# jianzongwu/betrayed-by-captions

Measured on AMD Instinct MI355X. Metric: images/sec (COCO-shaped 1024x1024, 100 queries, forward-only), higher is better.
Workload: dtype f32; 1 GPU; configs[1]: R50 + 100 queries, 1024x1024, batch 2/GPU, forward-only; global_batch=2, parallelism=replicas x1, precision=fp32 (parity mode, f16x3 MFMA), hip_graph=True, x3_overflow=False, library_fallbacks=0

## Files before the change

betrayed-by-captions_amd/_lib.py:

```python
import ctypes
import os

import torch

_HERE = os.path.dirname(os.path.abspath(__file__))
LIB_PATH = os.path.join(_HERE, 'lib', 'libcgg_hip.so')

CGG_F32 = 0
CGG_BF16 = 1

_c_int = ctypes.c_int
_c_vp = ctypes.c_void_p
_c_f = ctypes.c_float
_c_i64 = ctypes.c_int64

PROTOTYPES = {
    'cgg_version': (_c_int, []),
    'cgg_init': (_c_int, [_c_int]),
    'cgg_msda_forward_fused_vld': (_c_int, [_c_vp, _c_int, _c_vp, _c_vp, _c_vp, _c_int, _c_vp, _c_vp] + [_c_int] * 7 + [_c_vp]),
    'cgg_msda_backward_hostlevels_ws': (_c_int, [_c_vp, _c_int] + [_c_vp] * 8 + [_c_int] * 8 + [_c_vp, _c_i64, _c_vp, _c_vp]),
    'cgg_msda_backward_workspace_bytes': (_c_i64, [_c_vp, _c_vp] + [_c_int] * 7),
    'cgg_msda_read_levels': (_c_int, [_c_vp, _c_vp, _c_int, _c_int, _c_vp, _c_vp, _c_vp]),
    'cgg_last_error_string': (ctypes.c_char_p, []),
    'cgg_msda_forward': (_c_int, [_c_vp] * 6 + [_c_int] * 8 + [_c_vp]),
# ... 7 lines not shown
    'cgg_mask_logits': (_c_int, [_c_vp] * 5 + [_c_int] * 4 + [_c_vp]),
    'cgg_mask_logits_bits_astat': (_c_int, [_c_vp] * 3 + [_c_int] * 4 + [_c_vp]),
    'cgg_mask_logits_f32': (_c_int, [_c_vp] * 4 + [_c_int] * 4 + [_c_vp]),
    'cgg_mask_logits_backward_workspace_bytes': (_c_i64, [_c_int] * 4),
    'cgg_mask_logits_backward': (_c_int, [_c_vp] * 6 + [_c_int] * 5 + [_c_vp]),
    'cgg_attn_mask_fix_full_rows': (_c_int, [_c_vp, _c_int, _c_int, _c_vp]),
    'cgg_attn_mask_from_logits': (_c_int, [_c_vp, _c_vp] + [_c_int] * 5 + [_c_vp]),
    'cgg_masked_xattn_workspace_bytes': (_c_i64, [_c_int] * 5),
    'cgg_masked_xattn_forward': (_c_int, [_c_vp] * 5 + [_c_int] * 5 + [_c_f, _c_int, _c_vp]),
    'cgg_masked_xattn_forward_strided': (_c_int, [_c_vp, _c_vp, _c_int, _c_i64, _c_vp, _c_vp, _c_vp] + [_c_int] * 5 + [_c_f, _c_vp]),
    'cgg_masked_xattn_forward_x3': (_c_int, [_c_vp, _c_vp, _c_int, _c_i64, _c_vp, _c_vp, _c_vp] + [_c_int] * 5 + [_c_f, _c_vp]),
    'cgg_masked_xattn_forward_lse': (_c_int, [_c_vp] * 6 + [_c_int] * 5 + [_c_f, _c_int, _c_vp]),
    'cgg_masked_xattn_backward_workspace_bytes': (_c_i64, [_c_int] * 5),
    'cgg_masked_xattn_backward': (_c_int, [_c_vp] * 9 + [_c_int] * 5 + [_c_f, _c_int, _c_vp]),
    'cgg_masked_xattn_backward_x3': (_c_int, [_c_vp] * 10 + [_c_int] * 5 + [_c_f, _c_vp]),
    'cgg_window_attn_forward': (_c_int, [_c_vp] * 4 + [_c_int] * 7 + [_c_f, _c_vp]),
    'cgg_window_attn_backward_workspace_bytes': (_c_i64, [_c_int] * 5),
    'cgg_window_attn_backward': (_c_int, [_c_vp] * 7 + [_c_int] * 7 + [_c_f, _c_vp]),
    'cgg_grounding_pair_costs': (_c_int, [_c_vp] * 4 + [_c_int] * 5 + [_c_f, _c_vp]),
    'cgg_grounding_pair_costs_backward': (_c_int, [_c_vp] * 5 + [_c_int] * 5 + [_c_f, _c_vp]),
    'cgg_ce_rows_forward': (_c_int, [_c_vp] * 4 + [_c_int, _c_int, _c_i64, _c_i64, _c_int, _c_vp]),
    'cgg_ce_rows_backward': (_c_int, [_c_vp] * 4 + [_c_int, _c_int, _c_i64, _c_i64, _c_int, _c_vp]),
    'cgg_match_cost_rows': (_c_int, [_c_vp] * 4 + [_c_int, _c_int, _c_int, _c_vp]),
    'cgg_rle_encode_bitmasks': (_c_i64, [_c_vp, _c_int, _c_int, _c_int, _c_i64, _c_int, _c_int, _c_vp, _c_i64, _c_vp]),
    'cgg_masked_xattn_forward_bf16': (_c_int, [_c_vp] * 6 + [_c_int] * 5 + [_c_f, _c_int, _c_i64, _c_int, _c_vp]),
    'cgg_linear_rows': (_c_int, [_c_vp, _c_int, _c_vp, _c_vp, _c_vp, _c_int, _c_vp] + [_c_int] * 6 + [_c_vp]),
    'cgg_add_layernorm': (_c_int, [_c_vp] * 5 + [_c_int, _c_int, _c_f, _c_vp]),
    'cgg_linear_rows_packed_bytes': (_c_i64, [_c_int, _c_int]),
    'cgg_linear_rows_pack': (_c_int, [_c_vp, _c_vp, _c_int, _c_int, _c_vp]),
    'cgg_linear_rows_bf16': (_c_int, [_c_vp, _c_int, _c_vp, _c_vp, _c_vp, _c_int, _c_vp, _c_int, _c_vp, _c_vp, _c_f,
                                      _c_vp, _c_int, _c_vp, _c_int] + [_c_int] * 5 +
                             [_c_vp, _c_int, _c_int, _c_vp, _c_int, _c_int, _c_vp]),
    'cgg_decoder_tail_bf16': (_c_int, [_c_vp, _c_int, _c_i64, _c_int, _c_vp, _c_vp, _c_f, _c_vp, _c_int, _c_vp, _c_vp, _c_f] +
                              [_c_vp] * 12 + [_c_int, _c_int, _c_vp]),
    'cgg_self_attn_rows_bf16': (_c_int, [_c_vp, _c_int, _c_vp, _c_int, _c_vp] + [_c_int] * 4 + [_c_f, _c_vp]),
    'cgg_decoder_mid_bf16': (_c_int, [_c_vp, _c_int, _c_vp, _c_vp, _c_vp, _c_int, _c_vp, _c_vp, _c_f, _c_vp, _c_int] +
                             [_c_vp] * 5 + [_c_int, _c_int, _c_vp]),
    'cgg_decoder_ffn_bf16': (_c_int, [_c_vp, _c_int] + [_c_vp] * 5 + [_c_int] * 3 + [_c_vp]),
    'cgg_x3_packed_bytes': (_c_i64, [_c_int, _c_int]),
    'cgg_x3_pack': (_c_int, [_c_vp, _c_vp, _c_int, _c_int, _c_vp]),
    'cgg_linear_rows_x3': (_c_int, [_c_vp, _c_int, _c_vp, _c_vp, _c_vp, _c_int, _c_vp, _c_int, _c_vp, _c_vp, _c_f,
                                    _c_vp, _c_int, _c_vp, _c_int] + [_c_int] * 5 +
                           [_c_vp, _c_int, _c_int, _c_vp, _c_int, _c_int, _c_vp]),
    'cgg_decoder_tail_x3': (_c_int, [_c_vp, _c_int, _c_i64, _c_int, _c_vp, _c_vp, _c_f, _c_vp, _c_int, _c_vp, _c_vp, _c_f] +
                            [_c_vp] * 12 + [_c_int, _c_int, _c_vp]),
    'cgg_decoder_mid_x3': (_c_int, [_c_vp, _c_int, _c_vp, _c_vp, _c_vp, _c_int, _c_vp, _c_vp, _c_f, _c_vp, _c_int] +
                           [_c_vp] * 5 + [_c_int, _c_int, _c_vp]),
    'cgg_decoder_ffn_x3': (_c_int, [_c_vp, _c_int] + [_c_vp] * 5 + [_c_int] * 3 + [_c_vp]),
    'cgg_encoder_layer_tail_x3': (_c_int, [_c_vp] * 6 + [_c_f] + [_c_vp] * 6 + [_c_f, _c_vp, _c_int, _c_vp, _c_vp] +
                                  [_c_int] * 3 + [_c_vp]),
    'cgg_gemm_x3': (_c_int, [_c_vp, _c_int, _c_vp, _c_vp, _c_vp, _c_int, _c_vp, _c_int] + [_c_int] * 4 + [_c_vp]),
    'cgg_stem_conv7x7_x3_nchw': (_c_int, [_c_vp] * 4 + [_c_int] * 3 + [_c_vp]),
    'cgg_bias_relu_maxpool_nhwc_f32': (_c_int, [_c_vp] * 3 + [_c_int] * 4 + [_c_vp]),
    'cgg_gemm_x3_ex': (_c_int, [_c_vp, _c_int, _c_vp, _c_vp, _c_vp, _c_int, _c_int, _c_vp, _c_int, _c_vp, _c_int, _c_int] +
                       [_c_int] * 4 + [_c_vp]),
    'cgg_conv_x3_nhwc': (_c_int, [_c_vp] * 5 + [_c_int] * 10 + [_c_vp]),
    'cgg_gemm_x3s': (_c_int, [_c_vp, _c_int, _c_vp, _c_vp, _c_vp, _c_int, _c_int, _c_int, _c_vp, _c_int, _c_int] + [_c_int] * 4 + [_c_vp]),
    'cgg_gemm_x3s_batched': (_c_int, [_c_vp, _c_int, _c_int, _c_i64, _c_vp, _c_vp, _c_vp, _c_int, _c_int, _c_int, _c_vp, _c_int, _c_int] + [_c_int] * 4 + [_c_vp]),
    'cgg_conv_x3s_nhwc': (_c_int, [_c_vp] * 4 + [_c_int, _c_vp, _c_int] + [_c_int] * 10 + [_c_vp]),
    'cgg_x3a_encode': (_c_int, [_c_vp, _c_vp, _c_i64, _c_vp]),
    'cgg_x3a_decode': (_c_int, [_c_vp, _c_vp, _c_i64, _c_vp]),
    'cgg_x3_overflow_check': (_c_int, [_c_int, _c_vp, _c_vp]),
    'cgg_gemm_x3s_cfg': (_c_int, [_c_vp, _c_int, _c_vp, _c_vp, _c_vp, _c_int, _c_int, _c_int, _c_vp, _c_int, _c_int] + [_c_int] * 5 + [_c_vp]),
    'cgg_conv_x3s_nhwc_cfg': (_c_int, [_c_vp] * 4 + [_c_int, _c_vp, _c_int] + [_c_int] * 11 + [_c_vp]),
    'cgg_bias_relu_maxpool_nhwc_f32_x3a': (_c_int, [_c_vp] * 3 + [_c_int] * 4 + [_c_vp]),
    'cgg_group_norm_nhwc_f32_x3a': (_c_int, [_c_vp] * 4 + [_c_int] * 4 + [_c_f, _c_int, _c_vp, _c_int, _c_int, _c_i64, _c_int, _c_vp,
                                             _c_i64, _c_vp, _c_vp, _c_vp]),
    'cgg_encoder_layer_tail_x3a': (_c_int, [_c_vp] * 6 + [_c_f] + [_c_vp] * 6 + [_c_f, _c_vp, _c_int, _c_vp, _c_vp] +
                                   [_c_int] * 3 + [_c_vp]),
    'cgg_group_norm_nhwc_f32_stats': (_c_int, [_c_vp, _c_vp] + [_c_int] * 4 + [_c_vp]),
    'cgg_mask_feature_head_x3': (_c_int, [_c_vp] * 4 + [_c_f, _c_int] + [_c_vp] * 5 + [_c_int, _c_vp] + [_c_int] * 5 + [_c_vp]),
    'cgg_mask_feature_head_x3_cfg': (_c_int, [_c_vp] * 4 + [_c_f, _c_int] + [_c_vp] * 5 + [_c_int, _c_vp] + [_c_int] * 6 + [_c_vp]),
    'cgg_image_prep_u8': (_c_int, [_c_vp, _c_i64, _c_i64, _c_vp, _c_int, _c_vp, _c_vp, _c_vp, _c_int, _c_int, _c_vp, _c_int, _c_int, _c_vp]),
    'cgg_beam_step_workspace_bytes': (_c_i64, [_c_int] * 3),
    'cgg_beam_step': (_c_int, [_c_vp] + [_c_int] * 4 + [_c_vp] * 13 + [_c_int, _c_f, _c_int, _c_int, _c_int, _c_int, _c_vp]),
    'cgg_beam_step_passes': (_c_int, [_c_vp] + [_c_int] * 4 + [_c_vp] * 13 + [_c_int, _c_f, _c_int, _c_int, _c_int, _c_int, _c_int, _c_vp]),
    'cgg_wgrad_x3_workspace_bytes': (_c_i64, [_c_int] * 3),
    'cgg_wgrad_x3': (_c_int, [_c_vp, _c_int, _c_vp, _c_int, _c_vp, _c_vp] + [_c_int] * 3 + [_c_vp]),
    'cgg_wgrad_bias_x3': (_c_int, [_c_vp, _c_int, _c_vp, _c_int, _c_vp, _c_vp, _c_vp] + [_c_int] * 3 + [_c_vp]),
    'cgg_transpose_f32': (_c_int, [_c_vp, _c_vp, _c_int, _c_int, _c_int, _c_vp]),
    'cgg_nchw_to_nhwc_pad1_f32': (_c_int, [_c_vp, _c_vp] + [_c_int] * 4 + [_c_vp]),
    'cgg_topk_select': (_c_int, [_c_vp, _c_int, _c_int, _c_int, _c_int, _c_vp, _c_vp]),
    'cgg_absmax_f32': (_c_int, [_c_vp, _c_int, _c_int, _c_int, _c_vp, _c_vp]),
    'cgg_relu_bwd_absmax_f32': (_c_int, [_c_vp, _c_vp, _c_vp, ctypes.c_longlong, _c_vp, _c_vp]),
    'cgg_gemm_x3_bwd': (_c_int, [_c_vp, _c_int, _c_vp, _c_vp, _c_vp, _c_int, _c_vp, _c_int, _c_vp] + [_c_int] * 3 + [_c_vp]),
    'cgg_gemm_x3_scaled': (_c_int, [_c_vp, _c_int, _c_vp, _c_vp, _c_vp, _c_vp, _c_int, _c_vp, _c_int] + [_c_int] * 4 + [_c_vp]),
    'cgg_conv_x3_nhwc_scaled': (_c_int, [_c_vp] * 6 + [_c_int] * 10 + [_c_vp]),
    'cgg_wgrad_x3_scaled': (_c_int, [_c_vp, _c_int, _c_vp, _c_vp, _c_int, _c_vp, _c_vp, _c_vp] + [_c_int] * 3 + [_c_vp]),
    'cgg_layernorm_chain': (_c_int, [_c_vp, _c_int, _c_vp, _c_vp, _c_f, _c_vp, _c_int, _c_vp, _c_vp, _c_f, _c_vp, _c_vp,
                                     _c_vp, _c_int, _c_int, _c_int, _c_i64, _c_vp]),
    'cgg_msda_prologue': (_c_int, [_c_vp, _c_int, _c_vp, _c_vp, _c_vp, _c_vp] + [_c_int] * 5 + [_c_vp]),
    'cgg_msda_prologue_backward': (_c_int, [_c_vp, _c_vp, _c_vp, _c_int, _c_vp, _c_vp] + [_c_int] * 5 + [_c_vp]),
    'cgg_msda_forward_fused_bf16': (_c_int, [_c_vp] * 4 + [_c_int] + [_c_vp] * 2 + [_c_int] * 7 + [_c_vp]),
    'cgg_msda_forward_fused_bf16_hm': (_c_int, [_c_vp] * 4 + [_c_int] + [_c_vp] * 2 + [_c_int] * 7 + [_c_vp]),
    'cgg_decoder_kv_pack_k': (_c_int, [_c_vp, _c_vp, _c_int, _c_int, _c_vp]),
    'cgg_decoder_kv_proj_bf16': (_c_int, [_c_vp] * 7 + [_c_int] * 4 + [_c_vp]),
    'cgg_add_layernorm_backward_partials': (ctypes.c_int64, [_c_int]),
    'cgg_add_layernorm_backward': (_c_int, [_c_vp] * 5 + [_c_int, _c_vp, _c_f] + [_c_vp] * 3 + [_c_int, _c_int, _c_vp]),
    'cgg_add_layernorm_backward_amax': (_c_int, [_c_vp] * 5 + [_c_int, _c_vp, _c_f] + [_c_vp] * 4 + [_c_int, _c_int, _c_vp]),
    'cgg_bottleneck64_bf16': (_c_int, [_c_vp] * 8 + [_c_int] * 5 + [_c_vp]),
    'cgg_encoder_proj_pack': (_c_int, [_c_vp, _c_vp, _c_int, _c_int, _c_vp]),
    'cgg_encoder_proj_bf16': (_c_int, [_c_vp] * 3 + [_c_int] + [_c_vp] * 6 + [_c_int] * 5 + [_c_vp]),
    'cgg_encoder_ffn_ln_kv_bf16': (_c_int, [_c_vp] * 7 + [_c_f, _c_vp, _c_vp, _c_int, _c_vp, _c_int] + [_c_vp] * 3 +
                                   [_c_int] * 3 + [_c_vp]),
    'cgg_encoder_layer_tail_bf16': (_c_int, [_c_vp] * 6 + [_c_f] + [_c_vp] * 6 + [_c_f, _c_vp, _c_int, _c_vp, _c_vp, _c_int] +
                                    [_c_vp] * 3 + [_c_int] * 3 + [_c_vp]),
# ... 100 lines not shown
```

betrayed-by-captions_amd/backbones.py:

```python
import os

import torch
import torch.nn as nn

from . import ops, runtime
from .registry import BACKBONES

FROZEN_FOLDED = os.environ.get('CGG_FROZEN_FOLDED', '1') != '0'
X3_STEM = os.environ.get('CGG_X3_STEM', '1') != '0'


class Bottleneck(nn.Module):
    expansion = 4

    def __init__(self, inplanes, planes, stride=1, downsample=None, style='pytorch'):
        super().__init__()
        s1, s2 = (1, stride) if style == 'pytorch' else (stride, 1)
        self.conv1 = nn.Conv2d(inplanes, planes, 1, stride=s1, bias=False)
        self.bn1 = nn.BatchNorm2d(planes)
        self.conv2 = nn.Conv2d(planes, planes, 3, stride=s2, padding=1, bias=False)
        self.bn2 = nn.BatchNorm2d(planes)
        self.conv3 = nn.Conv2d(planes, planes * 4, 1, bias=False)
        self.bn3 = nn.BatchNorm2d(planes * 4)
        self.relu = nn.ReLU(inplace=True)
# ... 248 lines not shown
            if name == 'stem':
                return [fold(self.conv1, self.bn1, stem=True)]
            seq = []
            for blk in getattr(self, name):
                if blk.downsample is not None:
                    seq.append(fold(blk.downsample[0], blk.downsample[1]))
                seq.append(fold(blk.conv1, blk.bn1))
                seq.append(fold(blk.conv2, blk.bn2))
                if isinstance(blk, Bottleneck):
                    seq.append(fold(blk.conv3, blk.bn3))
            return seq

        cache = self.__dict__.setdefault('_fold_cache_x3', {})
        names = ['stem'] + list(self.res_layers if upto is None else self.res_layers[:upto])
        out = []
        for name in names:
            mods = [self.conv1, self.bn1] if name == 'stem' else [getattr(self, name)]
            tensors = [t for m in mods for t in list(m.parameters()) + list(m.buffers())]
            key = (sum(t._version for t in tensors), str(self.conv1.weight.device))
            hit = cache.get(name)
            if hit is None or hit[0] != key:
                with torch.no_grad():
                    hit = (key, stage_seq(name))
                cache[name] = hit
            out.extend(hit[1])
        return out

    def _x3_ok(self):
        def conv_ok(c):
            return (c.groups == 1 and tuple(c.dilation) == (1, 1) and c.kernel_size[0] == c.kernel_size[1]
                    and c.stride[0] == c.stride[1] and c.padding[0] == c.padding[1] and c.in_channels % 32 == 0 and c.bias is None
                    and c.out_channels % 8 == 0 and c.kernel_size[0] * c.kernel_size[1] <= 32)
        for name in self.res_layers:
            for blk in getattr(self, name):
                convs = [blk.conv1, blk.conv2] + ([blk.conv3] if isinstance(blk, Bottleneck) else [])
                if blk.downsample is not None:
                    if not (isinstance(blk.downsample[0], nn.Conv2d) and isinstance(blk.downsample[1], nn.BatchNorm2d)):
                        return False
                    convs.append(blk.downsample[0])
                if not all(conv_ok(c) for c in convs):
                    return False
        return self.conv1.bias is None

    def _forward_x3(self, x, upto=None):
        import torch.nn.functional as F
        x3a = runtime.x3a_enabled()
        seq = iter(self._folded_x3(upto))
        w, b = next(seq)
        mp, c1 = self.maxpool, self.conv1
        if ((mp.kernel_size, mp.stride, mp.padding, mp.dilation, mp.ceil_mode) == (3, 2, 1, 1, False) and x.dtype == torch.float32
                and x.is_contiguous() and tuple(c1.weight.shape) == (64, 3, 7, 7) and tuple(c1.stride) == (2, 2)
                and tuple(c1.padding) == (3, 3) and tuple(c1.dilation) == (1, 1) and X3_STEM):
            pk, sc = runtime.derived_cached('stem_packed_x3', (w,), lambda: ops.pack_stem_weight_x3(w))
            x = ops.bias_relu_maxpool_nhwc_f32(ops.stem_conv7x7_x3(x, pk, sc), b, x3a=x3a)
        else:
            x = F.conv2d(x.float(), w, b, stride=c1.stride, padding=c1.padding)
            x = mp(torch.relu_(x)).permute(0, 2, 3, 1).contiguous()
            if x3a:
                x = ops.x3a_encode(x)

        def conv(x, c, relu, res=None):
            wk, bias = next(seq)
            if x3a:
                return ops.conv_x3s_nhwc(x, wk, c.out_channels, c.kernel_size[0], c.stride[0], c.padding[0], bias, res=res, relu=relu)
            return ops.conv_x3_nhwc(x, wk, c.out_channels, c.kernel_size[0], c.stride[0], c.padding[0], bias, res=res, relu=relu)

        outs = []
        for i, name in enumerate(self.res_layers):
            if upto is not None and i >= upto:
                break
            for blk in getattr(self, name):
                identity = x if blk.downsample is None else conv(x, blk.downsample[0], False)
                y = conv(x, blk.conv1, True)
                if isinstance(blk, Bottleneck):
                    y = conv(y, blk.conv2, True)
                    x = conv(y, blk.conv3, True, identity)
                else:
                    x = conv(y, blk.conv2, True, identity)
            if i in self.out_indices:
                outs.append(x)
        if upto is not None:
            dec = (lambda t: ops.x3a_decode(t)) if x3a else (lambda t: t)
            return [dec(o) for o in outs], dec(x)
        if x3a and self.x3a_outputs:
            return tuple(ops.as_x3a(o.permute(0, 3, 1, 2)) for o in outs)
        if x3a:
            return tuple(ops.x3a_decode(o).permute(0, 3, 1, 2) for o in outs)
        return tuple(o.permute(0, 3, 1, 2) for o in outs)

    def forward(self, x):
        frozen_bn = all(not m.training for m in self.modules() if isinstance(m, nn.BatchNorm2d))
        if runtime.is_bf16() and not torch.is_grad_enabled() and frozen_bn and x.is_cuda:
            return self._forward_folded(x)
        if runtime.x3_enabled() and not torch.is_grad_enabled() and frozen_bn and x.is_cuda:
            if self._x3_ok():
                return self._forward_x3(x)
            runtime.note_fallback('ResNet', 'a convolution outside the implicit-GEMM rules (groups, dilation, C % 32, N % 8): MIOpen f32')
        outs = []
        frozen_nhwc = []
        first = 0
        xn = None
        if (FROZEN_FOLDED and runtime.x3_enabled() and torch.is_grad_enabled() and frozen_bn and x.is_cuda and self.frozen_stages >= 1
                and not x.requires_grad and self._x3_ok() and x.dtype == torch.float32
                and not any(p.requires_grad for n in self.res_layers[:self.frozen_stages] for p in getattr(self, n).parameters())
                and not any(p.requires_grad for p in list(self.conv1.parameters()) + list(self.bn1.parameters()))):
            with torch.no_grad():
                fouts, xf = self._forward_x3(x, upto=self.frozen_stages)
# ... 49 lines not shown
```

betrayed-by-captions_amd/csrc/stem_conv.hip:

```cpp
#include "x3.h"

typedef __attribute__((ext_vector_type(4))) uint32_t u32x4;

#define ST_TH 8
#define ST_TW 32
#define ST_IH (2 * ST_TH + 5)
#define ST_IW (2 * ST_TW + 5)
#define ST_IWP 72
#define ST_KS 11

template <bool X3>
__global__ __launch_bounds__(256) void cgg_stem_conv7x7_kernel(const float* __restrict__ img, const u32x4* __restrict__ wp,
                                                              void* __restrict__ out_, const float* __restrict__ wscale, int H,
                                                              int W, int Ho, int Wo) {
  constexpr int NP = X3 ? 2 : 1;
  constexpr int WFRAG = 2 * ST_KS * 64;
  constexpr int TILE_EL = (ST_IH + 1) * ST_IWP * 3;
  constexpr int OSZ = X3 ? 4 : 2;
  constexpr int LDS_BYTES = NP * (WFRAG * 16 + TILE_EL * 2) > (ST_TH * ST_TW * 64 * OSZ) ? NP * (WFRAG * 16 + TILE_EL * 2)
                                                                                           : (ST_TH * ST_TW * 64 * OSZ);
  __shared__ __attribute__((aligned(16))) unsigned char lds_raw[LDS_BYTES];
  u32x4* wl = reinterpret_cast<u32x4*>(lds_raw);
  uint16_t* tile = reinterpret_cast<uint16_t*>(lds_raw + NP * WFRAG * 16);
  uint16_t* obuf = reinterpret_cast<uint16_t*>(lds_raw);
  uint16_t* out = reinterpret_cast<uint16_t*>(out_);
  const int tid = threadIdx.x, lane = tid & 63, wave = tid >> 6;
  const int j = lane & 31, hi = lane >> 5;
  const int b = blockIdx.z, oy0 = blockIdx.y * ST_TH, ox0 = blockIdx.x * ST_TW;
  const int iy0 = 2 * oy0 - 3, ix0 = 2 * ox0 - 3;

  u32x4 wv[(NP * WFRAG + 255) / 256];
#pragma unroll
  for (int it = 0; it < (NP * WFRAG + 255) / 256; ++it) {
    const int i = tid + 256 * it;
    wv[it] = i < NP * WFRAG ? wp[i] : u32x4{0u, 0u, 0u, 0u};
  }

  const float* ib = img + (size_t)b * 3 * H * W;
  constexpr int NEL = (ST_IH + 1) * ST_IWP * 3;
  constexpr int NIT = (NEL + 255) / 256;
  float tv[NIT];
#pragma unroll
  for (int it = 0; it < NIT; ++it) {
    const int i = tid + 256 * it;
    const int c = i / ((ST_IH + 1) * ST_IWP);
    const int rem = i - c * ((ST_IH + 1) * ST_IWP);
    const int r = rem / ST_IWP, col = rem - r * ST_IWP;
    const int iy = iy0 + r, ix = ix0 + col;
    tv[it] = 0.f;
    if (i < NEL && r < ST_IH && col < ST_IW && iy >= 0 && iy < H && ix >= 0 && ix < W) tv[it] = ib[((size_t)c * H + iy) * W + ix];
  }
#pragma unroll
// ... 78 lines not shown
        *reinterpret_cast<f32x4*>(o32 + (((size_t)b * Ho + oy) * Wo + ox) * 64 + v4 * 4) =
            *reinterpret_cast<const f32x4*>(ob32 + pix * 64 + v4 * 4);
    }
    return;
  }
#pragma unroll
  for (int nt = 0; nt < 2; ++nt) {
    const int pix = (2 * wave + nt) * ST_TW + j;
#pragma unroll
    for (int mt = 0; mt < 2; ++mt)
#pragma unroll
      for (int gq = 0; gq < 4; ++gq) {
        const int ch = 32 * mt + 8 * gq + 4 * hi;
        *reinterpret_cast<uint2*>(obuf + pix * 64 + ch) =
            make_uint2(cgg_pack2(cgg_f2bf(acc[nt][mt][4 * gq]), cgg_f2bf(acc[nt][mt][4 * gq + 1])),
                       cgg_pack2(cgg_f2bf(acc[nt][mt][4 * gq + 2]), cgg_f2bf(acc[nt][mt][4 * gq + 3])));
      }
  }
  __syncthreads();
  for (int i = tid; i < ST_TH * ST_TW * 8; i += 256) {
    const int pix = i >> 3, v8 = i & 7;
    const int oy = oy0 + pix / ST_TW, ox = ox0 + pix % ST_TW;
    if (oy < Ho && ox < Wo)
      *reinterpret_cast<uint4*>(out + (((size_t)b * Ho + oy) * Wo + ox) * 64 + v8 * 8) =
          *reinterpret_cast<const uint4*>(obuf + pix * 64 + v8 * 8);
  }
}

extern "C" int64_t cgg_stem_conv7x7_packed_bytes(void) { return (int64_t)2 * ST_KS * 64 * 16; }

extern "C" int cgg_stem_conv7x7_nchw(const float* img, const void* w_packed, void* out, int B, int H, int W,
                                     cgg_stream_t stream) {
  CGG_REQUIRE(img && w_packed && out, CGG_EINVAL, "cgg_stem_conv7x7_nchw: null pointer");
  CGG_REQUIRE(B > 0 && H > 0 && W > 0, CGG_EINVAL, "cgg_stem_conv7x7_nchw: bad sizes");
  CGG_REQUIRE(cgg_aligned16(w_packed) && cgg_aligned16(out), CGG_EALIGN, "cgg_stem_conv7x7_nchw: alignment");
  const int Ho = (H - 1) / 2 + 1, Wo = (W - 1) / 2 + 1;
  hipLaunchKernelGGL(cgg_stem_conv7x7_kernel<false>, dim3((Wo + ST_TW - 1) / ST_TW, (Ho + ST_TH - 1) / ST_TH, B), dim3(256), 0,
                     (hipStream_t)stream, img, (const u32x4*)w_packed, out, (const float*)nullptr, H, W, Ho, Wo);
  CGG_CHECK_LAUNCH("cgg_stem_conv7x7_nchw");
  return CGG_OK;
}

extern "C" int cgg_stem_conv7x7_x3_nchw(const float* img, const void* w_packed, const float* wscale, float* out, int B, int H, int W,
                                        cgg_stream_t stream) {
  CGG_REQUIRE(img && w_packed && wscale && out, CGG_EINVAL, "cgg_stem_conv7x7_x3_nchw: null pointer");
  CGG_REQUIRE(B > 0 && H > 0 && W > 0, CGG_EINVAL, "cgg_stem_conv7x7_x3_nchw: bad sizes");
  CGG_REQUIRE(cgg_aligned16(w_packed) && cgg_aligned16(out) && cgg_aligned16(wscale), CGG_EALIGN, "cgg_stem_conv7x7_x3_nchw: alignment");
  const int Ho = (H - 1) / 2 + 1, Wo = (W - 1) / 2 + 1;
  hipLaunchKernelGGL(cgg_stem_conv7x7_kernel<true>, dim3((Wo + ST_TW - 1) / ST_TW, (Ho + ST_TH - 1) / ST_TH, B), dim3(256), 0,
                     (hipStream_t)stream, img, (const u32x4*)w_packed, (void*)out, wscale, H, W, Ho, Wo);
  CGG_CHECK_LAUNCH("cgg_stem_conv7x7_x3_nchw");
  return CGG_OK;
}
```

betrayed-by-captions_amd/ops.py:

```python
import ctypes
import os
import math

import torch

from . import _lib
from ._lib import CGG_BF16, CGG_F32, CggError, check, dev_ptr, stream_ptr

_WS_CACHE = {}

KERNEL_EVENTS = None


KERNEL_META = None


class _timed:
    def __init__(self, name, **meta):
        self.name = name
        self.meta = meta
        self.on = KERNEL_EVENTS is not None and not torch.cuda.is_current_stream_capturing()

    def __enter__(self):
        if self.on:
# ... 2048 lines not shown
    return out


def stem_conv7x7(img, packed):
    B, C, H, W = img.shape
    if C != 3 or img.dtype != torch.float32 or not img.is_contiguous():
        raise CggError('stem_conv7x7: img must be a contiguous (B, 3, H, W) float32 tensor')
    Ho, Wo = (H - 1) // 2 + 1, (W - 1) // 2 + 1
    y = torch.empty((B, Ho, Wo, 64), dtype=torch.bfloat16, device=img.device)
    check(_lib_().cgg_stem_conv7x7_nchw(dev_ptr(img), dev_ptr(packed), dev_ptr(y), B, H, W, stream_ptr(img.device)),
          'cgg_stem_conv7x7_nchw')
    return y


def pack_stem_weight_x3(w):
    if tuple(w.shape) != (64, 3, 7, 7):
        raise CggError(f'pack_stem_weight_x3: expected (64, 3, 7, 7), got {tuple(w.shape)}')
    wk = torch.zeros((64, 7, 8, 3), dtype=torch.float32, device=w.device)
    wk[:, :, :7, :] = w.detach().float().permute(0, 2, 3, 1)
    wk = torch.cat([wk.reshape(64, 168), torch.zeros((64, 8), dtype=torch.float32, device=w.device)], 1)
    amax = wk.abs().amax(1).clamp_min(1e-30)
    e = torch.floor(torch.log2(amax)) + 1
    s = torch.pow(2.0, 11 - e)
    ws = wk * s[:, None]
    hi = ws.to(torch.float16)
    lo = (ws - hi.float()).to(torch.float16)
    frag = lambda t: t.view(2, 32, 11, 2, 8).permute(0, 2, 3, 1, 4).contiguous().view(torch.uint8).reshape(-1)
    packed = torch.cat([frag(hi), frag(lo)])
    assert packed.numel() == 2 * _lib_().cgg_stem_conv7x7_packed_bytes()
    return packed, (1.0 / (s * 16.0)).float().contiguous()


def stem_conv7x7_x3(img, packed, wscale):
    B, C, H, W = img.shape
    if C != 3 or img.dtype != torch.float32 or not img.is_contiguous():
        raise CggError('stem_conv7x7_x3: img must be a contiguous (B, 3, H, W) float32 tensor')
    Ho, Wo = (H - 1) // 2 + 1, (W - 1) // 2 + 1
    y = torch.empty((B, Ho, Wo, 64), dtype=torch.float32, device=img.device)
    check(_lib_().cgg_stem_conv7x7_x3_nchw(dev_ptr(img), dev_ptr(packed), dev_ptr(wscale, 'wscale', torch.float32), dev_ptr(y), B, H, W,
                                           stream_ptr(img.device)), 'cgg_stem_conv7x7_x3_nchw')
    return y


def bias_relu_maxpool_nhwc_f32(x, bias, x3a=False):
    B, H, W, C = x.shape
    Ho, Wo = (H - 1) // 2 + 1, (W - 1) // 2 + 1
    y = torch.empty((B, Ho, Wo, C), dtype=torch.float32, device=x.device)
    fn = _lib_().cgg_bias_relu_maxpool_nhwc_f32_x3a if x3a else _lib_().cgg_bias_relu_maxpool_nhwc_f32
    rc = fn(dev_ptr(x, 'x', torch.float32), dev_ptr(bias, 'bias', torch.float32), dev_ptr(y), B, H, W, C, stream_ptr(x.device))
    check(rc, 'cgg_bias_relu_maxpool_nhwc_f32')
    return y


def linear_sum_assignment_batch(costs):
    if not costs:
        return []
    flat = torch.cat([c.detach().to(device='cpu', dtype=torch.float32).contiguous().reshape(-1) for c in costs]) \
        if len(costs) > 1 else costs[0].detach().to(device='cpu', dtype=torch.float32).contiguous().reshape(-1)
    nr = [int(c.shape[0]) for c in costs]
    nc = [int(c.shape[1]) for c in costs]
    sizes = [min(a, b) for a, b in zip(nr, nc)]
    total = sum(sizes)
    rows = torch.empty((max(total, 1),), dtype=torch.int64)
    cols = torch.empty((max(total, 1),), dtype=torch.int64)
    rc = _lib_().cgg_linear_sum_assignment_f32(ctypes.c_void_p(flat.data_ptr()) if flat.numel() else None, len(costs),
                                               _int_array(nr), _int_array(nc), ctypes.c_void_p(rows.data_ptr()),
                                               ctypes.c_void_p(cols.data_ptr()))
    check(rc, 'cgg_linear_sum_assignment_f32')
    out, o = [], 0
    for n in sizes:
        out.append((rows[o:o + n], cols[o:o + n]))
        o += n
    return out


def point_sample_planes(planes, index, points):
    N, H, W = planes.shape
    rows, P, _ = points.shape
    out = torch.empty((rows, P), dtype=torch.float32, device=planes.device)
    if rows == 0:
        return out
    check(_lib_().cgg_point_sample_planes(dev_ptr(planes, 'planes', torch.float32), dev_ptr(index, 'index', torch.int32),
                                          dev_ptr(points.contiguous(), 'points', torch.float32), dev_ptr(out), N, H, W, rows, P,
                                          stream_ptr(planes.device)), 'cgg_point_sample_planes')
    return out


class _PointSampleRowsFn(torch.autograd.Function):

    @staticmethod
    def forward(ctx, planes, points):
        planes = planes.contiguous()
        points = points.contiguous()
        rows, H, W = planes.shape
        idx = torch.arange(rows, dtype=torch.int32, device=planes.device)
        ctx.save_for_backward(points)
        ctx.shape = (rows, H, W)
        return point_sample_planes(planes, idx, points)

    @staticmethod
    def backward(ctx, gout):
        (points,) = ctx.saved_tensors
        rows, H, W = ctx.shape
        if rows and rows <= 65535 and W <= 16384:
            gp = torch.empty((rows, H, W), dtype=torch.float32, device=gout.device)
            check(_lib_().cgg_point_sample_planes_backward_rows(dev_ptr(gout.contiguous().float(), 'grad', torch.float32),
# ... 205 lines not shown
```

include/cgg_hip.h:

```cpp
#ifndef CGG_HIP_H_
#define CGG_HIP_H_

#include <stdint.h>

#ifdef __cplusplus
extern "C" {
#endif

#define CGG_VERSION 100

#define CGG_OK 0
#define CGG_EINVAL (-1)
#define CGG_EUNSUPPORTED (-2)
#define CGG_EALIGN (-3)
#define CGG_ELIBRARY (-4)

#define CGG_F32 0
#define CGG_BF16 1
#define CGG_F32_BF16MFMA 2
#define CGG_F32_X3 3

typedef void* cgg_stream_t;

int cgg_version(void);
// ... 146 lines not shown
                        float* y, float* yp, float* z, int rows, int N, int nsum, int64_t plane,
                        cgg_stream_t stream);

int cgg_decoder_tail_bf16(const float* planes, int nsum, int64_t plane_stride, int ld, const float* gamma_a,
                          const float* beta_a, float eps_a, const float* pos, int pos_rows, const float* gamma_b,
                          const float* beta_b, float eps_b, const void* w1, const float* b1, const void* w2,
                          const float* b2, const void* w3, const float* b3, const void* wq, const float* bq, float* y,
                          float* yp, float* mask_embed, float* qn, int M, int C, cgg_stream_t stream);

int cgg_decoder_mid_bf16(const float* core, int ldc, const void* wo, const float* bo, const float* res, int ldr,
                         const float* gamma, const float* beta, float eps, const float* pos, int pos_rows,
                         const void* wqkv, const float* bqkv, float* x1, float* q, float* kv, int M, int C,
                         cgg_stream_t stream);

int cgg_decoder_ffn_bf16(const float* x, int ldx, const void* w1, const float* b1, const void* w2, const float* b2,
                         float* planes, int M, int C, int F, cgg_stream_t stream);

int64_t cgg_x3_packed_bytes(int N, int K);
int cgg_x3_pack(const float* w, void* packed, int N, int K, cgg_stream_t stream);
int cgg_linear_rows_x3(const float* x, int ldx, const void* w_x3, const float* bias, const float* res,
                       int ldr, float* y, int ldy, const float* ln_gamma, const float* ln_beta, float ln_eps,
                       const float* pos, int pos_rows, float* yp, int ldyp, int M, int N, int K, int relu_cols,
                       int ksplit, const float* x2, int ldx2, int x2_col, float* y2, int ldy2, int y2_col,
                       cgg_stream_t stream);
int cgg_decoder_tail_x3(const float* planes, int nsum, int64_t plane_stride, int ld, const float* gamma_a,
                        const float* beta_a, float eps_a, const float* pos, int pos_rows, const float* gamma_b,
                        const float* beta_b, float eps_b, const void* w1, const float* b1, const void* w2,
                        const float* b2, const void* w3, const float* b3, const void* wq, const float* bq, float* y,
                        float* yp, float* mask_embed, float* qn, int M, int C, cgg_stream_t stream);
int cgg_decoder_mid_x3(const float* core, int ldc, const void* wo, const float* bo, const float* res, int ldr,
                       const float* gamma, const float* beta, float eps, const float* pos, int pos_rows,
                       const void* wqkv, const float* bqkv, float* x1, float* q, float* kv, int M, int C,
                       cgg_stream_t stream);
int cgg_decoder_ffn_x3(const float* x, int ldx, const void* w1, const float* b1, const void* w2, const float* b2,
                       float* planes, int M, int C, int F, cgg_stream_t stream);

int cgg_group_norm_nhwc_f32(const float* x, const float* gamma, const float* beta, void* ws, int B, int HW, int C, int groups,
                            float eps, int relu, const float* up_src, int up_h, int up_w, int64_t up_bstride, int W,
                            float* y32, int64_t y32_bstride, void* y16, const float* pos, void* yp16, int64_t y16_bstride,
                            cgg_stream_t stream);
int cgg_pack_mask_feature_nhwc_f32_x3(const float* feat, void* const* hi_host, void* const* lo_host, const int* pools_host,
                                      int n, int B, int C, int H, int W, cgg_stream_t stream);
int cgg_point_sample_nhwc_x3(const float* feat, const float* pts, void* hi, void* lo, int B, int H, int W, int C, int P_total,
                             int P_group, cgg_stream_t stream);
int cgg_encoder_layer_tail_x3(const float* a32, const float* x32, const void* wo_x3, const float* bo, const float* gamma0,
                              const float* beta0, float eps0, const void* w1_x3, const float* b1, const void* w2_x3,
                              const float* b2, const float* gamma1, const float* beta1, float eps1, const float* pos,
                              int pos_rows, float* y32, float* yp32, int M, int C, int F, cgg_stream_t stream);
int cgg_gemm_x3(const float* a, int lda, const void* w_x3, const float* bias, const float* res, int ldr, float* out, int ldc,
                int M, int N, int K, int relu, cgg_stream_t stream);
int cgg_stem_conv7x7_x3_nchw(const float* img, const void* w_packed, const float* wscale, float* out, int B, int H, int W,
                             cgg_stream_t stream);
int cgg_bias_relu_maxpool_nhwc_f32(const float* x, const float* bias, float* y, int B, int H, int W, int C, cgg_stream_t stream);
int cgg_gemm_x3_ex(const float* a, int lda, const void* w_x3, const float* bias, const float* res, int ldr, int res_mod, float* out,
                   int ldc, float* out2, int ldc2, int col2, int M, int N, int K, int relu, cgg_stream_t stream);
int cgg_conv_x3_nhwc(const float* x, const void* w_x3, const float* bias, const float* res, float* out, int B, int H, int W,
                     int C, int N, int KH, int KW, int stride, int pad, int relu, cgg_stream_t stream);

int cgg_gemm_x3s(const void* a_x3a, int lda, const void* w_x3, const float* bias, const void* res, int ldr, int res_fmt,
                 int res_mod, void* out, int ldc, int out_fmt, int M, int N, int K, int relu, cgg_stream_t stream);
int cgg_gemm_x3s_batched(const void* a_x3a, int lda, int rows_per_image, int64_t a_bstride, const void* w_x3, const float* bias,
                         const void* res, int ldr, int res_fmt, int res_mod, void* out, int ldc, int out_fmt, int M, int N, int K,
                         int relu, cgg_stream_t stream);
int cgg_conv_x3s_nhwc(const void* x_x3a, const void* w_x3, const float* bias, const void* res, int res_fmt, void* out,
                      int out_fmt, int B, int H, int W, int C, int N, int KH, int KW, int stride, int pad, int relu,
                      cgg_stream_t stream);
int cgg_x3a_encode(const float* x, void* out_x3a, int64_t n, cgg_stream_t stream);
int cgg_x3a_decode(const void* x_x3a, float* out, int64_t n, cgg_stream_t stream);
int cgg_x3_overflow_check(int reset, int* value_host, cgg_stream_t stream);
int cgg_gemm_x3s_cfg(const void* a_x3a, int lda, const void* w_x3, const float* bias, const void* res, int ldr, int res_fmt,
                     int res_mod, void* out, int ldc, int out_fmt, int M, int N, int K, int relu, int cfg, cgg_stream_t stream);
int cgg_conv_x3s_nhwc_cfg(const void* x_x3a, const void* w_x3, const float* bias, const void* res, int res_fmt, void* out,
                          int out_fmt, int B, int H, int W, int C, int N, int KH, int KW, int stride, int pad, int relu, int cfg,
                          cgg_stream_t stream);
int cgg_bias_relu_maxpool_nhwc_f32_x3a(const float* x, const float* bias, void* y_x3a, int B, int H, int W, int C,
                                       cgg_stream_t stream);
int cgg_group_norm_nhwc_f32_x3a(const float* x, const float* gamma, const float* beta, void* ws, int B, int HW, int C, int groups,
                                float eps, int relu, const void* up_src_x3a, int up_h, int up_w, int64_t up_bstride, int W,
                                void* y_x3a, int64_t y_bstride, const float* pos, void* yp_x3a, cgg_stream_t stream);

int64_t cgg_group_norm_nhwc_backward_workspace_bytes(int B, int HW, int groups);
int cgg_group_norm_nhwc_f32_backward(const float* x, const float* y, const float* dy, const float* stats, const float* gamma, void* ws,
                                     int B, int HW, int C, int groups, float eps, int relu, float* dx, float* tot, float* dlo, int lo_h,
                                     int lo_w, int W, int dx_padded, cgg_stream_t stream);
int cgg_group_norm_nhwc_f32_padout(const float* x, const float* gamma, const float* beta, void* ws, int B, int HW, int C, int groups,
                                   float eps, int relu, const float* up_src, int up_h, int up_w, int64_t up_bstride, int W,
                                   float* y_padded, cgg_stream_t stream);
int cgg_encoder_layer_tail_x3a(const float* a32, const void* x_x3a, const void* wo_x3, const float* bo, const float* gamma0,
                               const float* beta0, float eps0, const void* w1_x3, const float* b1, const void* w2_x3,
                               const float* b2, const float* gamma1, const float* beta1, float eps1, const float* pos,
                               int pos_rows, void* y_x3a, void* yp_x3a, int M, int C, int F, cgg_stream_t stream);
int cgg_group_norm_nhwc_f32_stats(const float* x, void* ws, int B, int HW, int C, int groups, cgg_stream_t stream);
int cgg_mask_feature_head_x3(const float* z, const void* gn_ws, const float* gamma, const float* beta, float eps, int groups,
                             const void* w_x3, const float* bias, void* const* hi_host, void* const* lo_host, const int* pools_host,
                             int n, float* mf, int B, int H, int W, int C, int N, cgg_stream_t stream);
int cgg_mask_feature_head_x3_cfg(const float* z, const void* gn_ws, const float* gamma, const float* beta, float eps, int groups,
                                 const void* w_x3, const float* bias, void* const* hi_host, void* const* lo_host,
                                 const int* pools_host, int n, float* mf, int B, int H, int W, int C, int N, int cfg,
                                 cgg_stream_t stream);

#define CGG_IMAGE_PREP_MAX_DIM 65535
int cgg_image_prep_u8(const uint8_t* staged, int64_t staged_bytes, int64_t table_offset, const int32_t* table_host, int B,
                      const float* mean, const float* std, const float* pad_val, int to_rgb, int pad_before_norm, float* out, int Hb,
                      int Wb, cgg_stream_t stream);

#define CGG_BEAM_STEP_MAX_BEAM 8
// ... 150 lines not shown
```

Baseline: 400.1 images/sec.

## Fuse stem 7x7 conv with bias, ReLU and 3x3 maxpool in one kernel

Adds a single HIP kernel that computes the stem 7x7 stride-2 convolution with x3 MFMA on a tile, including a halo, stages the conv output in LDS, then applies bias, ReLU and the 3x3/2 maxpool and writes pooled NHWC output (optionally x3a-encoded). This avoids writing the full-resolution conv output to global memory and reading it back in a separate pool kernel. The cost is recomputing halo conv pixels at tile edges and a larger LDS footprint per block.

```diff
diff --git a/betrayed-by-captions_amd/_lib.py b/betrayed-by-captions_amd/_lib.py
--- a/betrayed-by-captions_amd/_lib.py
+++ b/betrayed-by-captions_amd/_lib.py
@@ -83,6 +83,7 @@
     'cgg_gemm_x3': (_c_int, [_c_vp, _c_int, _c_vp, _c_vp, _c_vp, _c_int, _c_vp, _c_int] + [_c_int] * 4 + [_c_vp]),
     'cgg_stem_conv7x7_x3_nchw': (_c_int, [_c_vp] * 4 + [_c_int] * 3 + [_c_vp]),
     'cgg_bias_relu_maxpool_nhwc_f32': (_c_int, [_c_vp] * 3 + [_c_int] * 4 + [_c_vp]),
+    'cgg_stem_conv7x7_pool_x3_nchw': (_c_int, [_c_vp] * 5 + [_c_int] * 4 + [_c_vp]),
     'cgg_gemm_x3_ex': (_c_int, [_c_vp, _c_int, _c_vp, _c_vp, _c_vp, _c_int, _c_int, _c_vp, _c_int, _c_vp, _c_int, _c_int] +
                        [_c_int] * 4 + [_c_vp]),
     'cgg_conv_x3_nhwc': (_c_int, [_c_vp] * 5 + [_c_int] * 10 + [_c_vp]),
diff --git a/betrayed-by-captions_amd/backbones.py b/betrayed-by-captions_amd/backbones.py
--- a/betrayed-by-captions_amd/backbones.py
+++ b/betrayed-by-captions_amd/backbones.py
@@ -324,7 +324,7 @@
                 and x.is_contiguous() and tuple(c1.weight.shape) == (64, 3, 7, 7) and tuple(c1.stride) == (2, 2)
                 and tuple(c1.padding) == (3, 3) and tuple(c1.dilation) == (1, 1) and X3_STEM):
             pk, sc = runtime.derived_cached('stem_packed_x3', (w,), lambda: ops.pack_stem_weight_x3(w))
-            x = ops.bias_relu_maxpool_nhwc_f32(ops.stem_conv7x7_x3(x, pk, sc), b, x3a=x3a)
+            x = ops.stem_conv7x7_pool_x3(x, pk, sc, b, x3a=x3a)
         else:
             x = F.conv2d(x.float(), w, b, stride=c1.stride, padding=c1.padding)
             x = mp(torch.relu_(x)).permute(0, 2, 3, 1).contiguous()
diff --git a/betrayed-by-captions_amd/csrc/stem_conv.hip b/betrayed-by-captions_amd/csrc/stem_conv.hip
--- a/betrayed-by-captions_amd/csrc/stem_conv.hip
+++ b/betrayed-by-captions_amd/csrc/stem_conv.hip
@@ -1,3 +1,4 @@
+#include <type_traits>
 #include "x3.h"
 
 typedef __attribute__((ext_vector_type(4))) uint32_t u32x4;
@@ -182,3 +183,214 @@
   CGG_CHECK_LAUNCH("cgg_stem_conv7x7_x3_nchw");
   return CGG_OK;
 }
+
+#define SP_PH 4
+#define SP_PW 16
+#define SP_CH (2 * SP_PH + 1)
+#define SP_CW (2 * SP_PW + 1)
+#define SP_IH (2 * SP_CH + 5)
+#define SP_IW (2 * SP_CW + 5)
+#define SP_IWP 72
+#define SP_OOB 0xFFFFFF00u
+#define SP_NT 320
+static_assert(SP_IWP >= 2 * (SP_CW - 1) + 8 && SP_IWP >= SP_IW, "stem tile: fragment reads must stay inside the padded row");
+static_assert(SP_CH - 1 == 8 && SP_CW - 1 == 32 && SP_CH <= 32, "stem tile: 4 waves x 2 body rows of one n-tile each");
+
+__global__ __launch_bounds__(SP_NT) void cgg_stem_conv7x7_pool_x3_kernel(const float* __restrict__ img, const u32x4* __restrict__ wp,
+                                                                        const float* __restrict__ wscale,
+                                                                        const f32x4* __restrict__ bias, f32x4* __restrict__ y, int H,
+                                                                        int W, int Ho, int Wo, int Hp, int Wp, int x3a,
+                                                                        int* __restrict__ flag) {
+  constexpr int WFRAG = 2 * ST_KS * 64;
+  constexpr int TILE_EL = (SP_IH + 1) * SP_IWP * 3;
+  constexpr int STAGE_BYTES = SP_CH * SP_CW * 64 * 4;
+  constexpr int LDS_BYTES = 2 * (WFRAG * 16 + TILE_EL * 2) > STAGE_BYTES ? 2 * (WFRAG * 16 + TILE_EL * 2) : STAGE_BYTES;
+  __shared__ __attribute__((aligned(16))) unsigned char lds_raw[LDS_BYTES];
+  u32x4* wl = reinterpret_cast<u32x4*>(lds_raw);
+  uint16_t* tile = reinterpret_cast<uint16_t*>(lds_raw + 2 * WFRAG * 16);
+  float* ob32 = reinterpret_cast<float*>(lds_raw);
+  const int tid = threadIdx.x, lane = tid & 63, wave = tid >> 6;
+  const int j = lane & 31, hi = lane >> 5;
+  const int b = blockIdx.z, py0 = blockIdx.y * SP_PH, px0 = blockIdx.x * SP_PW;
+  const int iy0 = 4 * py0 - 5, ix0 = 4 * px0 - 5;
+
+  constexpr int WIT = (2 * WFRAG + SP_NT - 1) / SP_NT;
+  u32x4 wv[WIT];
+#pragma unroll
+  for (int it = 0; it < WIT; ++it) {
+    const int i = tid + SP_NT * it;
+    wv[it] = i < 2 * WFRAG ? wp[i] : u32x4{0u, 0u, 0u, 0u};
+  }
+
+  const float* ib = img + (size_t)b * 3 * H * W;
+  const __amdgpu_buffer_rsrc_t irsrc = __builtin_amdgcn_make_buffer_rsrc(const_cast<float*>(ib), 0, (uint32_t)(3 * H * W) * 4u, 0x00020000);
+  constexpr int RP = SP_IH + 1;
+  constexpr int NIT = (TILE_EL + SP_NT - 1) / SP_NT;
+  static_assert(SP_NT == 4 * SP_IWP + 32 && SP_NT < RP * SP_IWP, "stem tile: the element walk below");
+  auto walk = [](int& c, int& r, int& col) {
+    col += 32;
+    r += 4;
+    if (col >= SP_IWP) {
+      col -= SP_IWP;
+      ++r;
+    }
+    if (r >= RP) {
+      r -= RP;
+      ++c;
+    }
+  };
+  float tv[NIT];
+  {
+    int c = 0, r = tid / SP_IWP, col = tid - (tid / SP_IWP) * SP_IWP;
+#pragma unroll
+    for (int it = 0; it < NIT; ++it) {
+      const int iy = iy0 + r, ix = ix0 + col;
+      const bool in = (SP_NT * (it + 1) <= TILE_EL || c < 3) && r < SP_IH && col < SP_IW && (unsigned)iy < (unsigned)H &&
+                      (unsigned)ix < (unsigned)W;
+      tv[it] = __builtin_bit_cast(float, __builtin_amdgcn_raw_buffer_load_b32(irsrc, in ? (uint32_t)((c * H + iy) * W + ix) * 4u : SP_OOB, 0, 0));
+      walk(c, r, col);
+    }
+  }
+  {
+    int c = 0, r = tid / SP_IWP, col = tid - (tid / SP_IWP) * SP_IWP;
+#pragma unroll
+    for (int it = 0; it < NIT; ++it) {
+      if (SP_NT * (it + 1) <= TILE_EL || c < 3) {
+        uint16_t h, l;
+        cgg_x3_split1(tv[it], h, l);
+        tile[(r * SP_IWP + col) * 3 + c] = h;
+        tile[TILE_EL + (r * SP_IWP + col) * 3 + c] = l;
+      }
+      walk(c, r, col);
+    }
+  }
+#pragma unroll
+  for (int it = 0; it < WIT; ++it) {
+    const int i = tid + SP_NT * it;
+    if (i < 2 * WFRAG) wl[i] = wv[it];
+  }
+  __syncthreads();
+
+  int lr[2], lc[2];
+  bool keep[2];
+#pragma unroll
+  for (int nt = 0; nt < 2; ++nt) {
+    const bool col_tile = wave == 4 && nt == 1;
+    lr[nt] = wave < 4 ? 1 + 2 * wave + nt : (col_tile ? (j < SP_CH ? j : SP_CH - 1) : 0);
+    lc[nt] = col_tile ? 0 : 1 + j;
+    keep[nt] = !col_tile || j < SP_CH;
+  }
+  f32x16 acc[2][2];
+#pragma unroll
+  for (int nt = 0; nt < 2; ++nt)
+#pragma unroll
+    for (int mt = 0; mt < 2; ++mt)
+#pragma unroll
+      for (int r = 0; r < 16; ++r) acc[nt][mt][r] = 0.f;
+#pragma unroll
+  for (int ks = 0; ks < ST_KS; ++ks) {
+    const int g = 2 * ks + hi;
+    const int ky = g / 3, part = g - 3 * ky;
+#pragma unroll
+    for (int nt = 0; nt < 2; ++nt) {
+      const uint16_t* src = tile + ((2 * lr[nt] + ky) * SP_IWP + 2 * lc[nt]) * 3 + 8 * part;
+      const uint32_t* s32 = reinterpret_cast<const uint32_t*>(src);
+      const u32x4 bv = {s32[0], s32[1], s32[2], s32[3]};
+      const uint32_t* l32 = reinterpret_cast<const uint32_t*>(src + TILE_EL);
+      const u32x4 bl = {l32[0], l32[1], l32[2], l32[3]};
+#pragma unroll
+      for (int mt = 0; mt < 2; ++mt)
+        cgg_x3_mfma(acc[nt][mt], wl[(mt * ST_KS + ks) * 64 + lane], wl[WFRAG + (mt * ST_KS + ks) * 64 + lane], bv, bl);
+    }
+  }
+  __syncthreads();
+#pragma unroll
+  for (int nt = 0; nt < 2; ++nt) {
+    const int pix = lr[nt] * SP_CW + lc[nt];
+    if (keep[nt]) {
+#pragma unroll
+      for (int mt = 0; mt < 2; ++mt)
+#pragma unroll
+        for (int gq = 0; gq < 4; ++gq) {
+          const int ch = 32 * mt + 8 * gq + 4 * hi;
+          const f32x4 sc = *reinterpret_cast<const f32x4*>(wscale + ch);
+          *reinterpret_cast<f32x4*>(ob32 + pix * 64 + (((ch >> 2) ^ (lc[nt] & 7)) << 2)) =
+              f32x4{acc[nt][mt][4 * gq] * sc[0], acc[nt][mt][4 * gq + 1] * sc[1], acc[nt][mt][4 * gq + 2] * sc[2],
+                    acc[nt][mt][4 * gq + 3] * sc[3]};
+        }
+    }
+  }
+  __syncthreads();
+  if (tid >= SP_PW * 16) return;
+  const int c = tid & 15, pc = tid >> 4;
+  const int px = px0 + pc;
+  if (px >= Wp) return;
+  const float ninf = -__builtin_inff();
+  const f32x4 bv = bias[c];
+  int coff[3];
+  bool xin[3];
+#pragma unroll
+  for (int dx = 0; dx < 3; ++dx) {
+    const int l = 2 * pc + dx;
+    coff[dx] = l * 64 + ((c ^ (l & 7)) << 2);
+    xin[dx] = (unsigned)(2 * px - 1 + dx) < (unsigned)Wo;
+  }
+  const bool interior = py0 > 0 && 2 * (py0 + SP_PH) - 1 < Ho && px0 > 0 && 2 * (px0 + SP_PW) - 1 < Wo;
+  auto pool_rows = [&](auto all_in) {
+#pragma unroll
+    for (int pr = 0; pr < SP_PH; ++pr) {
+      const int py = py0 + pr;
+      if (py >= Hp) break;
+      f32x4 v[9];
+#pragma unroll
+      for (int t = 0; t < 9; ++t) v[t] = *reinterpret_cast<const f32x4*>(ob32 + (2 * pr + t / 3) * (SP_CW * 64) + coff[t % 3]);
+      f32x4 m = {ninf, ninf, ninf, ninf};
+#pragma unroll
+      for (int t = 0; t < 9; ++t) {
+        if constexpr (decltype(all_in)::value) {
+#pragma unroll
+          for (int k = 0; k < 4; ++k) m[k] = fmaxf(m[k], v[t][k]);
+        } else {
+          const bool in = (unsigned)(2 * py - 1 + t / 3) < (unsigned)Ho && xin[t % 3];
+#pragma unroll
+          for (int k = 0; k < 4; ++k) m[k] = in ? fmaxf(m[k], v[t][k]) : m[k];
+        }
+      }
+      f32x4 o;
+#pragma unroll
+      for (int k = 0; k < 4; ++k) o[k] = fmaxf(m[k] + bv[k], 0.f);
+      const size_t oi = (((size_t)b * Hp + py) * Wp + px) * 16 + c;
+      if (!x3a) {
+        y[oi] = o;
+        continue;
+      }
+      uint2 h, l;
+      cgg_x3_split4(o, h, l);
+      uint2* yo = reinterpret_cast<uint2*>(y) + (oi >> 1) * 4 + (oi & 1);
+      yo[0] = h;
+      yo[2] = l;
+      if (!(fmaxf(fmaxf(o[0], o[1]), fmaxf(o[2], o[3])) * CGG_X3_ASCALE <= CGG_X3A_MAX)) atomicOr(flag, 1);
+    }
+  };
+  if (interior) pool_rows(std::true_type{});
+  else pool_rows(std::false_type{});
+}
+
+int* cgg_x3_overflow_flag_ptr();
+
+extern "C" int cgg_stem_conv7x7_pool_x3_nchw(const float* img, const void* w_packed, const float* wscale, const float* bias, void* y,
+                                             int B, int H, int W, int x3a, cgg_stream_t stream) {
+  CGG_REQUIRE(img && w_packed && wscale && bias && y, CGG_EINVAL, "cgg_stem_conv7x7_pool_x3_nchw: null pointer");
+  CGG_REQUIRE(B > 0 && B <= 65535 && H > 0 && W > 0 && (x3a == 0 || x3a == 1), CGG_EINVAL, "cgg_stem_conv7x7_pool_x3_nchw: bad sizes");
+  CGG_REQUIRE(cgg_aligned16(w_packed) && cgg_aligned16(wscale) && cgg_aligned16(bias) && cgg_aligned16(y), CGG_EALIGN,
+              "cgg_stem_conv7x7_pool_x3_nchw: alignment");
+  const int Ho = (H - 1) / 2 + 1, Wo = (W - 1) / 2 + 1;
+  const int Hp = (Ho - 1) / 2 + 1, Wp = (Wo - 1) / 2 + 1;
+  CGG_REQUIRE((Hp + SP_PH - 1) / SP_PH <= 65535 && (long long)3 * H * W * 4 < (long long)SP_OOB, CGG_EINVAL,
+              "cgg_stem_conv7x7_pool_x3_nchw: bad sizes");
+  hipLaunchKernelGGL(cgg_stem_conv7x7_pool_x3_kernel, dim3((Wp + SP_PW - 1) / SP_PW, (Hp + SP_PH - 1) / SP_PH, B), dim3(SP_NT), 0,
+                     (hipStream_t)stream, img, (const u32x4*)w_packed, wscale, (const f32x4*)bias, (f32x4*)y, H, W, Ho, Wo, Hp, Wp,
+                     x3a, x3a ? cgg_x3_overflow_flag_ptr() : nullptr);
+  CGG_CHECK_LAUNCH("cgg_stem_conv7x7_pool_x3_nchw");
+  return CGG_OK;
+}
diff --git a/betrayed-by-captions_amd/ops.py b/betrayed-by-captions_amd/ops.py
--- a/betrayed-by-captions_amd/ops.py
+++ b/betrayed-by-captions_amd/ops.py
@@ -2124,6 +2124,21 @@
     return y
 
 
+def stem_conv7x7_pool_x3(img, packed, wscale, bias, x3a=False):
+    B, C, H, W = img.shape
+    if C != 3 or img.dtype != torch.float32 or not img.is_contiguous():
+        raise CggError('stem_conv7x7_pool_x3: img must be a contiguous (B, 3, H, W) float32 tensor')
+    if bias.numel() != 64:
+        raise CggError('stem_conv7x7_pool_x3: bias must have 64 elements')
+    Ho, Wo = (H - 1) // 2 + 1, (W - 1) // 2 + 1
+    y = torch.empty((B, (Ho - 1) // 2 + 1, (Wo - 1) // 2 + 1, 64), dtype=torch.float32, device=img.device)
+    rc = _lib_().cgg_stem_conv7x7_pool_x3_nchw(dev_ptr(img), dev_ptr(packed), dev_ptr(wscale, 'wscale', torch.float32),
+                                               dev_ptr(bias, 'bias', torch.float32), dev_ptr(y), B, H, W, int(bool(x3a)),
+                                               stream_ptr(img.device))
+    check(rc, 'cgg_stem_conv7x7_pool_x3_nchw')
+    return y
+
+
 def linear_sum_assignment_batch(costs):
     if not costs:
         return []
diff --git a/include/cgg_hip.h b/include/cgg_hip.h
--- a/include/cgg_hip.h
+++ b/include/cgg_hip.h
@@ -222,6 +222,8 @@
 int cgg_stem_conv7x7_x3_nchw(const float* img, const void* w_packed, const float* wscale, float* out, int B, int H, int W,
                              cgg_stream_t stream);
 int cgg_bias_relu_maxpool_nhwc_f32(const float* x, const float* bias, float* y, int B, int H, int W, int C, cgg_stream_t stream);
+int cgg_stem_conv7x7_pool_x3_nchw(const float* img, const void* w_packed, const float* wscale, const float* bias, void* y, int B,
+                                  int H, int W, int x3a, cgg_stream_t stream);
 int cgg_gemm_x3_ex(const float* a, int lda, const void* w_x3, const float* bias, const float* res, int ldr, int res_mod, float* out,
                    int ldc, float* out2, int ldc2, int col2, int M, int N, int K, int relu, cgg_stream_t stream);
 int cgg_conv_x3_nhwc(const float* x, const void* w_x3, const float* bias, const float* res, float* out, int B, int H, int W,
```

New measurement: 401.1 images/sec, median of 3. Within noise of the previous version (+0.2%).
